# shinshoji01/Style-Restricted_GAN

Hardware: AMD Instinct MI355X
Metric: images/sec G+D+E train step, CelebA 128x128 bs=32/GPU (higher is better)
Workload: dtype f32; 1 GPU; SRGAN-nopretrain (03-train) G+D+E train step, 128x128, bs=32/GPU, k=5, fp32, E trainable (BASELINE configs[1]); global_batch=32, unrolled_k=5, parallelism=dp1, graph_fallback=False, graph_segments=1, ranks_seen=1, execution=hipGraph replay of the captured step

## Files before the change

style-restricted_gan_amd/csrc/conv_igemm.hip:

```cpp
#include <algorithm>
#include <cstdlib>
#include <cstring>
#include <map>
#include <mutex>
#include <string>
#include <vector>
#include "common.h"
#include "pack_device.h"

namespace srgan {

struct ProfSlot { hipEvent_t a, b; int kid; double flops; };
static bool g_prof_on = false;
static std::vector<ProfSlot> g_prof_slots;
static std::vector<std::pair<hipEvent_t, hipEvent_t>> g_prof_pool;
static size_t g_prof_next = 0;
static const char* const kProfNames[] = {
    "igemm_kernel<128,128,2,2,gen>", "igemm_kernel<128,128,2,2,vec>", "igemm_kernel<128,64,2,2,gen>", "igemm_kernel<128,64,2,2,vec>",
    "igemm_kernel<128,32,4,1,gen>",  "igemm_kernel<128,32,4,1,vec>",  "igemm_kernel<64,64,2,2,gen>",  "igemm_kernel<64,64,2,2,vec>",
    "wgrad_kernel<gen>", "wgrad_kernel<vec>", "igemm_kernel<256,128,4,2,gen>", "igemm_kernel<256,128,4,2,vec>",
    "igemm_kernel<256,64,4,2,gen>", "igemm_kernel<256,64,4,2,vec>", "wino_kernel", "wino_wgrad_kernel", "wino_kernel<4x4s2>", "wino_wgrad_kernel<4x4s2>",
    "wino43_kernel", "wino43_input_kernel", "rgbin_conv_kernel", "rgb_wgrad_kernel", "wino43_wgrad_kernel", "wino43_dy_kernel",
    "halo16_kernel", "halo16_wgrad_kernel", "halo16s2_wgrad_kernel", "halo16t_kernel", "rgbout_conv_kernel", "halo16s_kernel",
    "in_stats_partial", "in_apply", "in_bwd_partial", "in_bwd_apply", "in_fwd_slab", "in_bwd_slab", "igemm16_kernel",
// ... 1639 lines not shown
  const long long f = (long long)npad_for(M_f, d->O) * Kf;
  const int s = d->stride;
  const int Ty = (int)ceil_div(d->kh, s), Tx = (int)ceil_div(d->kw, s);
  const long long Kd = round_up((long long)Ty * Tx * d->O, BK);
  const long long g = (long long)s * s * round_up(d->I, 128) * Kd;
  size_t bytes = (size_t)((f > g ? f : g) * sizeof(float));
  if (rowconv_applicable(d)) bytes = std::max(bytes, rowconv_packed_elems(d) * sizeof(float));
  {
    srgan_conv_desc f;
    long long w_off;
    if (narrow_dgrad_desc(d, &f, &w_off) && rowconv_applicable(&f)) bytes = std::max(bytes, rowconv_packed_elems(&f) * sizeof(float));
  }
  if (wino_applicable(d, 0)) bytes = std::max(bytes, wino_packed_bytes(d, 0));
  if (wino_applicable(d, 1)) bytes = std::max(bytes, wino_packed_bytes(d, 1));
  if (d->I == 3 || d->O == 3) bytes = std::max(bytes, (size_t)d->kh * ((d->kw * 3 + 1) & ~1) * std::max(d->I, d->O) * sizeof(float));
  return bytes;
}

}
}

using namespace srgan;

namespace srgan { static size_t conv_splitk_bytes(const srgan_conv_desc* d, int kind); }

extern "C" size_t srgan_conv2d_workspace(const srgan_conv_desc* d) {
  if (validate(d) != 0) return 0;
  size_t bytes = pack_bytes(d);
  if (d->pad_mode == SRGAN_PAD_REFLECT)
    bytes += (size_t)d->N * (d->Hi + 2 * d->pad) * (d->Wi + 2 * d->pad) * d->I * sizeof(float);
  bytes += 256 + std::max(conv_splitk_bytes(d, 0), conv_splitk_bytes(d, 1));
  bytes = std::max(bytes, (size_t)round_up((long long)pack_bytes(d), 256) + std::max(wino_scratch_bytes(d, 0), wino_scratch_bytes(d, 1)));
  WgradPlan w = plan_wgrad(d);
  if (wino_wgrad_applicable(d)) wino_wgrad_slab(d, &w.splits, &w.Cdpad, &w.NNpad);
  if (rgb_wgrad_kind(d) >= 0) rgb_wgrad_slab(d, &w.splits, &w.Cdpad, &w.NNpad);
  size_t wg = (size_t)w.splits * w.Cdpad * w.NNpad * sizeof(float);
  size_t cs = (size_t)1024 * d->O * sizeof(float);
  if (wg + cs > bytes) bytes = wg + cs;
  if (narrow_applicable(d)) bytes = std::max(bytes, narrow_workspace(d) + cs);
  {
    Wino43WgradGeom wg43{};
    if (wino43_wgrad_geometry(d, &wg43)) bytes = std::max(bytes, (size_t)round_up((long long)(wg43.slab_bytes + cs), 256) + wg43.z_bytes);
  }
  return bytes + 4096;
}

namespace srgan {
enum FwdPath { PATH_IGEMM = 0, PATH_NARROW = 1, PATH_WAVE = 2, PATH_DENSE = 3, PATH_WINO = 4, PATH_ROWCONV = 5, PATH_RGBIN = 6 };

static bool rowconv_applicable(const srgan_conv_desc* d) {
  static const bool off = SRGAN_AB_SET("SRGAN_NO_ROWCONV");
  return !off && d->O == 3 && d->kh == 7 && d->kw == 7 && d->stride == 1 && d->pad_mode == SRGAN_PAD_ZERO && (d->I % BK) == 0 &&
         d->Wo >= 64 && d->Ho >= 8 && (long long)d->N * d->Ho * d->Wi * 21 < (1LL << 30);
}
constexpr int RC_N = 21, RC_NPAD = 32;
// ... 322 lines not shown
    long long w_off;
    narrow_dgrad_desc(d, &f, &w_off);
    if (rowconv_applicable(&f)) return rowconv_run(&f, dy, wp, nullptr, dx, st);
    return narrow_fwd_packed(&f, dy, wp, nullptr, dx, st);
  }
  if (g.rgbin) {
    srgan_conv_desc f;
    long long w_off;
    rgbin_dgrad_desc(d, &f, &w_off);
    return rgbin_run(&f, dy, wp, nullptr, dx, SRGAN_ACT_NONE, 0.f, st);
  }
  if (g.narrow_s2) {
    for (int ph = 0; ph < 4; ++ph) {
      srgan_conv_desc f;
      long long w_off;
      int px;
      size_t po;
      if (!narrow_s2_phase(d, ph >> 1, ph & 1, &f, &w_off, &px, &po)) { set_error("narrow stride-2 dgrad: phase geometry"); return -1; }
      if (int e = narrow_fwd_strided(&f, px, dy, wp + po, dx, d->Hi, d->Wi, ph >> 1, ph & 1, st)) return e;
    }
    return 0;
  }
  if (g.wino) {
    if (int e = wino_run(d, 1, dy, wp, nullptr, g.p.dst, SRGAN_ACT_NONE, 0.f, g.reflect ? nullptr : scratch, st,
                         g.reflect ? nullptr : res, res_done, false, (g.reflect || res) ? nullptr : mask, mask_slope, mask_done)) return e;
  } else {
    float* slab = scratch ? (g.reflect ? scratch + round_up((long long)d->N * g.Hd * g.Wd * d->I, 64) : scratch) : nullptr;
    if (int e = run_igemm(g.p, g.phases, st, conv_flops(d), slab)) return e;
  }
  if (g.reflect) {
    long long n = (long long)d->N * d->Hi * d->Wi * d->I;
    hipLaunchKernelGGL(reflect_fold_kernel<false>, dim3((unsigned)std::min<long long>(ceil_div(n, 256), 8192)), dim3(256), 0, st,
                       (const float*)scratch, dx, d->N, d->Hi, d->Wi, d->I, d->pad);
    return check_launch("reflect_fold_kernel");
  }
  return 0;
}
}

extern "C" int srgan_conv2d_fwd(const srgan_conv_desc* d, const float* x, const float* w, const float* bias,
                                float* y, int act, float slope, void* ws, size_t ws_bytes, void* stream) {
  if (int e = validate(d)) return e;
  SRGAN_REQUIRE(x && w && y && ws, "conv2d_fwd: null pointer");
  SRGAN_REQUIRE(ws_bytes >= srgan_conv2d_workspace(d), "conv2d_fwd: workspace too small");
  hipStream_t st = as_stream(stream);
  if (int e = fwd_pack(d, act, w, (float*)ws, st)) return e;
  return fwd_run(d, x, (const float*)ws, bias, y, act, slope, (float*)ws + round_up((long long)(pack_bytes(d) / sizeof(float)), 64), st);
// ... 721 lines not shown
```

style-restricted_gan_amd/csrc/conv_wino.hip:

```cpp
#include <algorithm>
#include <cstdlib>
#include <type_traits>
#include "common.h"
#include "pack_device.h"

#ifndef WINO_EXP
#define WINO_EXP 0
#endif

namespace srgan {

constexpr int WT = 64;
constexpr int WNB = 64;
constexpr int WC = 8;

__device__ __forceinline__ auto uniform_rsrc(const float* base, unsigned bytes) {
  const unsigned long long a = reinterpret_cast<unsigned long long>(base);
  const unsigned lo = __builtin_amdgcn_readfirstlane((unsigned)a), hi = __builtin_amdgcn_readfirstlane((unsigned)(a >> 32));
  float* q = reinterpret_cast<float*>(((unsigned long long)hi << 32) | lo);
  return __builtin_amdgcn_make_buffer_rsrc(q, 0, __builtin_amdgcn_readfirstlane(bytes), 0x00020000);
}



// ... 652 lines not shown
}

static bool wino_disabled() {
  static const bool off = SRGAN_AB_SET("SRGAN_NO_WINOGRAD");
  return off;
}
double wino_threshold_scale() {
  const char* e = std::getenv("SRGAN_WINOGRAD_THRESHOLD_SCALE");
  return e ? std::atof(e) : 1.0;
}
static bool wino43_disabled() {
  static const bool off = SRGAN_AB_SET("SRGAN_NO_WINOGRAD43");
  return off;
}
static bool wino_s2_disabled() {
  static const bool off = SRGAN_AB_SET("SRGAN_NO_WINOGRAD_S2");
  return off;
}
static bool wino42_disabled() {
  static const bool off = SRGAN_AB_SET("SRGAN_NO_WINOGRAD42");
  return off;
}

static int wino_variant(const srgan_conv_desc* d, int kind) {
  if (compute_bf16()) {
    if (halo16_applicable(d, kind)) return 4;
    if (kind == 1 && halo16t_applicable(d)) return 5;
    return kind == 0 && halo16s_applicable(d) ? 6 : 0;
  }
  if (wino_disabled()) return 0;

  const int C = kind == 0 ? d->I : d->O, N = kind == 0 ? d->O : d->I;
  if (C % (2 * WC) != 0 || C < 32 || N < 32 || N % 4 != 0) return 0;
  const long long src_elems = (long long)d->N * (kind == 0 ? (long long)d->Hi * d->Wi * d->I : (long long)d->Ho * d->Wo * d->O);
  if (src_elems >= (1LL << 29)) return 0;
  if (d->kh == 3 && d->kw == 3 && d->stride == 1 && d->pad == 1) {
    if (d->Hi < 3 || d->Wi < 3) return 0;
    const int ho = kind == 0 ? d->Ho : d->Hi, wo = kind == 0 ? d->Wo : d->Wi;
    if (!wino43_disabled() && d->pad_mode == SRGAN_PAD_ZERO && ho % 4 == 0 && wo % 4 == 0 && N % 32 == 0 && C % 32 == 0) {
      const long long b43 = ceil_div((long long)d->N * (ho / 4) * (wo / 4), 64) * (N / 32);
      if (b43 >= 50 * wino_threshold_scale()) return 3;
    }
    const long long blocks = ceil_div((long long)d->N * ceil_div(ho, 2) * ceil_div(wo, 2), WT) * ceil_div(N, WNB);
    return blocks >= 100 * wino_threshold_scale() ? 1 : 0;
  }
  if (d->kh == 4 && d->kw == 4 && d->stride == 2 && d->pad == 1 && d->pad_mode == SRGAN_PAD_ZERO && !wino_s2_disabled()) {
    if ((d->Hi & 1) || (d->Wi & 1)) return 0;
    const long long dst_elems = (long long)d->N * (kind == 0 ? (long long)d->Ho * d->Wo * d->O : (long long)d->Hi * d->Wi * d->I);
    if (!wino42_disabled() && d->Ho % 4 == 0 && d->Wo % 4 == 0 && N % 64 == 0 && C % 16 == 0 && dst_elems < (1LL << 30) &&
        (kind == 1 || C <= 128)) {
      const long long b42 = ceil_div((long long)d->N * (d->Ho / 4) * (d->Wo / 4), 32) * (N / 64) * (kind == 1 ? 4 : 1);
      if (b42 >= 120 * wino_threshold_scale()) return 7;
    }
    const long long th = ceil_div(d->Ho, 3), tw = ceil_div(d->Wo, 3);
    const double eff = (double)d->Ho * d->Wo / (9.0 * th * tw);
    if (eff * 2.25 < 1.5) return 0;
    const long long blocks = ceil_div((long long)d->N * th * tw, WT) * ceil_div(N, WNB) * (kind == 1 ? 4 : 1);
    return blocks >= 120 * wino_threshold_scale() ? 2 : 0;
  }
  return 0;
}

bool wino_applicable(const srgan_conv_desc* d, int kind) { return wino_variant(d, kind) != 0; }

static void wino_dims(const srgan_conv_desc* d, int kind, int* C, int* N, int* n_tiles, int* nchunk, int* phases) {
  const int v = wino_variant(d, kind);
  *C = kind == 0 ? d->I : d->O;
  *N = kind == 0 ? d->O : d->I;
  *n_tiles = v == 7 ? *N / 64 : (v >= 4) ? 1 : v == 3 ? *N / 32 : (int)ceil_div(*N, WNB);
  *nchunk = v == 7 ? (kind == 0 ? 4 : 1) * (*C / 16) : (v >= 4) ? *C / 32 : (v == 2 && kind == 0 ? 4 : 1) * (*C / WC);
  *phases = ((v == 2 || v == 7) && kind == 1) ? 4 : 1;
}

size_t wino_packed_bytes(const srgan_conv_desc* d, int kind) {
  int C, N, n_tiles, nchunk, phases;
  wino_dims(d, kind, &C, &N, &n_tiles, &nchunk, &phases);
  if (wino_variant(d, kind) == 4) return halo16_packed_bytes(d);
  if (wino_variant(d, kind) == 6) return halo16s_packed_bytes(d);
  if (wino_variant(d, kind) == 5) return halo16t_packed_bytes(d);
  if (wino_variant(d, kind) == 3) return (size_t)n_tiles * nchunk * (36 * 256) * sizeof(float);
  if (wino_variant(d, kind) == 7) return (size_t)phases * n_tiles * nchunk * (25 * 1024) * sizeof(float);
  return (size_t)phases * n_tiles * nchunk * 8192 * sizeof(float);
}

size_t wino_scratch_bytes(const srgan_conv_desc* d, int kind) {
  if (wino_variant(d, kind) != 3) return 0;
  const int ho = kind == 0 ? d->Ho : d->Hi, wo = kind == 0 ? d->Wo : d->Wi;
  return wino43_scratch_floats((long long)d->N * (ho / 4) * (wo / 4), kind == 0 ? d->I : d->O) * sizeof(float);
}

bool wino43_wgrad_geometry(const srgan_conv_desc* d, Wino43WgradGeom* g) {
  static const bool off = SRGAN_AB_SET("SRGAN_NO_WINOGRAD43_WGRAD");
  if (off || wino_variant(d, 0) != 3 || d->I % 64 != 0 || d->O % 32 != 0) return false;
  const long long T = (long long)d->N * (d->Ho / 4) * (d->Wo / 4);
  const long long ntc = ceil_div(T, 64) * 8;
  const int tiles = (d->O / 32) * (d->I / 64);
  long long splits = std::max(1, 256 / tiles);
  long long cps = std::max<long long>(2, ceil_div(ntc, splits));
  if (ntc % cps == 1) ++cps;
  splits = ceil_div(ntc, cps);
  if (ntc < 2 || ntc - (splits - 1) * cps < 2) return false;
  g->NB = d->N; g->H = d->Ho; g->W = d->Wo; g->C = d->I; g->O = d->O; g->ntc = (int)ntc;
  g->splits = (int)splits; g->chunks_per_split = (int)cps;
  g->v_bytes = wino_scratch_bytes(d, 0);
  g->z_bytes = (size_t)(d->O / 32) * ntc * 36 * 256 * sizeof(float);
  g->slab_bytes = (size_t)splits * d->O * 9 * d->I * sizeof(float);
  return g->v_bytes < (1ULL << 32) && g->z_bytes < (1ULL << 32);
}

void wino_pack_params(const srgan_conv_desc* d, int kind, const float* w, float* dst, WinoPackParams* out) {
  WinoPackParams q{};
  int C, N;
  wino_dims(d, kind, &C, &N, &q.n_tiles, &q.nchunk, &q.phases);
  q.variant = wino_variant(d, kind);
  q.w = w; q.dst = dst; q.sO = d->sO; q.sI = d->sI; q.sH = d->sH; q.sW = d->sW; q.N = N; q.C = C; q.kind = kind;
  q.no_block = std::getenv("SRGAN_PACK_ITEM_PATH") != nullptr ? 1 : 0;
  *out = q;
}

int wino_pack(const srgan_conv_desc* d, int kind, const float* w, float* dst, hipStream_t st) {
  WinoPackParams q{};
  wino_pack_params(d, kind, w, dst, &q);
  const long long total = wino_pack_total(q);
  hipLaunchKernelGGL(wino_pack_kernel, dim3((unsigned)std::min<long long>(ceil_div(total, 256), 4096)), dim3(256), 0, st, q);
  return check_launch("wino_pack_kernel");
}

bool wino43_fwd_applicable(const srgan_conv_desc* d) { return wino_variant(d, 0) == 3; }
bool wino43_dgrad_applicable(const srgan_conv_desc* d) { return d->pad_mode == SRGAN_PAD_ZERO && wino_variant(d, 1) == 3; }

int wino_run(const srgan_conv_desc* d, int kind, const float* src, const float* packed, const float* bias, float* dst,
             int act, float slope, float* scratch, hipStream_t st, const float* res, bool* res_done, bool v_ready,
             const float* mask, float mask_slope, bool* mask_done) {
  if (res_done) *res_done = false;
  if (mask_done) *mask_done = false;
  WinoParams p{};
  p.act = act; p.slope = slope;
  int C, N, phases;
  wino_dims(d, kind, &C, &N, &p.n_tiles, &p.nchunk, &phases);
  const int variant = wino_variant(d, kind);
  SRGAN_REQUIRE(variant != 0, "winograd: layer not applicable");
  if (variant == 6) {
    SRGAN_REQUIRE(!v_ready && !res && !mask, "halo16s: no prepared image, skip tensor or mask on this path");
    return halo16s_run(d, src, packed, bias, dst, act, slope, conv_flops_of(d), st);
  }
  if (variant == 5) {
    SRGAN_REQUIRE(!v_ready && !bias && act == SRGAN_ACT_NONE, "halo16t: plain transposed product only");
    return halo16t_run(d, src, packed, dst, conv_flops_of(d), st);
  }
  if (variant == 4) {
    SRGAN_REQUIRE(!v_ready, "halo16: no transformed-input image on this path");
    if (res_done) *res_done = res != nullptr;
    return halo16_run(d, kind, src, packed, bias, res, dst, act, slope, conv_flops_of(d), st);
  }
  const bool reflect = d->pad_mode == SRGAN_PAD_REFLECT;
  p.src = src; p.u = packed; p.bias = bias; p.dst = dst;
  p.NB = d->N; p.C = C; p.Cd = N; p.cpp = C / WC;
  int ot = 2;
  if (variant == 1 || variant == 3) {
    if (kind == 0) {
      p.H = d->Hi; p.W = d->Wi; p.Ho = d->Ho; p.Wo = d->Wo; p.pad = d->pad; p.reflect = reflect ? 1 : 0;
    } else {
      p.H = d->Ho; p.W = d->Wo; p.reflect = 0;
      p.pad = reflect ? 2 : 2 - d->pad;
      p.Ho = d->Ho + 2 * p.pad - 2; p.Wo = d->Wo + 2 * p.pad - 2;
    }
    if (variant == 3) { ot = 4; p.TH = p.Ho / 4; p.TW = p.Wo / 4; }
    else { p.TH = (p.Ho + 1) / 2; p.TW = (p.Wo + 1) / 2; }
  } else {
    ot = variant == 7 ? 4 : 3;
    p.pad = d->pad; p.reflect = 0;
    if (kind == 0) { p.H = d->Hi; p.W = d->Wi; p.Ho = d->Ho; p.Wo = d->Wo; }
    else { p.H = d->Ho; p.W = d->Wo; p.Ho = d->Hi; p.Wo = d->Wi; }
    p.TH = (int)ceil_div(d->Ho, ot); p.TW = (int)ceil_div(d->Wo, ot);
    if (variant == 7) p.cpp = C / 16;
  }
  (void)ot;
  const long long T = (long long)p.NB * p.TH * p.TW;
  SRGAN_REQUIRE(T < (1LL << 30), "winograd: too many tiles");
  p.T = (int)T;
  p.m_tiles = (int)ceil_div(T, variant == 7 ? 32 : WT);
  const long long grid = (long long)p.m_tiles * p.n_tiles;
  SRGAN_REQUIRE(grid < (1LL << 31), "winograd: grid too large");
  if (variant == 3) {
    SRGAN_REQUIRE(p.pad == 1 && p.Ho == p.H && p.Wo == p.W && p.nchunk >= 2 && p.Cd % 32 == 0 && p.C % 32 == 0,
                  "winograd F(4,3): geometry");
    SRGAN_REQUIRE(scratch, "winograd F(4,3): no scratch for the transformed input");
    p.res = res;
    if (res_done) *res_done = res != nullptr;
    wino43_launch(p, scratch, grid, conv_flops_of(d), st, v_ready);
    return check_launch("wino43_kernel");
  }
  SRGAN_REQUIRE(!v_ready, "winograd: a prepared V image only serves the F(4x4,3x3) path");
  if (variant == 7) {
    SRGAN_REQUIRE(p.pad == 1 && p.nchunk >= 2 && p.Cd % 64 == 0 && p.C % 16 == 0 && d->Ho % 4 == 0 && d->Wo % 4 == 0, "winograd F(4,2): geometry");
    if (kind == 1 && mask) {
      p.mask = mask; p.mask_slope = mask_slope;
      if (mask_done) *mask_done = true;
    }
    return wino42_launch(p, kind, grid, kind == 1 && mask != nullptr, conv_flops_of(d), st);
  }
  ProfToken tok = prof_begin(variant == 1 ? 14 : 16, conv_flops_of(d), st);
  if (variant == 1) hipLaunchKernelGGL(wino_kernel<0>, dim3((unsigned)grid), dim3(512), 0, st, p);
  else if (kind == 0) hipLaunchKernelGGL(wino_kernel<1>, dim3((unsigned)grid), dim3(512), 0, st, p);
  else if (mask) {
    p.mask = mask; p.mask_slope = mask_slope;
    if (mask_done) *mask_done = true;
    hipLaunchKernelGGL((wino_kernel<2, true>), dim3((unsigned)grid, 4), dim3(512), 0, st, p);
  } else hipLaunchKernelGGL(wino_kernel<2>, dim3((unsigned)grid, 4), dim3(512), 0, st, p);
  prof_end(tok, st);
  return check_launch("wino_kernel");
}
// ... 88 lines not shown
```

style-restricted_gan_amd/csrc/conv_wino43.hip:

```cpp
#include <algorithm>
#include <cstdlib>
#include <type_traits>
#include "common.h"
#include "pack_device.h"

namespace srgan {

__device__ __forceinline__ void bt6(f32x4& x0, f32x4& x1, f32x4& x2, f32x4& x3, f32x4& x4, f32x4& x5) {
  const f32x4 a = x4 - 4.f * x2, b = x3 - 4.f * x1, c = x4 - x2, e = x3 - x1;
  const f32x4 n0 = 4.f * x0 - 5.f * x2 + x4, n5 = 4.f * x1 - 5.f * x3 + x5;
  x0 = n0; x1 = a + b; x2 = a - b; x3 = c + 2.f * e; x4 = c - 2.f * e; x5 = n5;
}

__device__ __forceinline__ void at6(float m0, float m1, float m2, float m3, float m4, float m5, float* y) {
  const float s1 = m1 + m2, d1 = m1 - m2, s2 = m3 + m4, d2 = m3 - m4;
  y[0] = m0 + s1 + s2;
  y[1] = d1 + 2.f * d2;
  y[2] = s1 + 4.f * s2;
  y[3] = d1 + 8.f * d2 + m5;
}

__device__ __forceinline__ auto uniform_rsrc43(const float* base, unsigned bytes) {
  const unsigned long long a = reinterpret_cast<unsigned long long>(base);
  const unsigned lo = __builtin_amdgcn_readfirstlane((unsigned)a), hi = __builtin_amdgcn_readfirstlane((unsigned)(a >> 32));
  float* q = reinterpret_cast<float*>(((unsigned long long)hi << 32) | lo);
  return __builtin_amdgcn_make_buffer_rsrc(q, 0, __builtin_amdgcn_readfirstlane(bytes), 0x00020000);
}

constexpr int W4T = 64;
constexpr int W4N = 32;
constexpr int W4C = 8;
constexpr int W4BLK = 36 * 512;

__global__ __launch_bounds__(512) void wino43_input_kernel(WinoParams p, float* vimg) {
  const int tid = threadIdx.x, lane = tid & 63, wave = tid >> 6;
  const int cgs = p.C / 32;
  int m_tile, cg;
  if ((p.m_tiles & 7) == 0) {
    const int xcd = blockIdx.x & 7, k = blockIdx.x >> 3;
    cg = k % cgs;
    m_tile = (k / cgs) * 8 + xcd;
  } else {
    m_tile = blockIdx.x / cgs;
    cg = blockIdx.x - m_tile * cgs;
  }
  const int quad = lane & 7, tl = wave * 8 + (lane >> 3);
  const int t = m_tile * W4T + tl;
  const bool tv = t < p.T;
  const int tt = tv ? t : 0;
  const int per = p.TH * p.TW;
  const int nb = tt / per;
  const int r0 = tt - nb * per;
  const int ty = r0 / p.TW, tx = r0 - ty * p.TW;
  const int Y = 4 * ty, X = 4 * tx;
  const int RS = p.W * p.C * 4, CS = p.C * 4;
  const auto rs_x = uniform_rsrc43(p.src, (unsigned)((size_t)p.NB * p.H * p.W * p.C * 4));
  constexpr unsigned kOutside = 0x80000000u;
  const unsigned base = (unsigned)(((nb * p.H + Y) * p.W + X) * p.C + cg * 32 + quad * 4) * 4u;
  const bool rok[3] = {Y > 0, true, Y + 4 < p.H};
  const bool cok[3] = {X > 0, true, X + 4 < p.W};
  const int rdl[3] = {-RS, 0, RS}, cdl[3] = {-CS, 0, CS};
  unsigned voff[3][3];
#pragma unroll
  for (int a = 0; a < 3; ++a)
#pragma unroll
    for (int b = 0; b < 3; ++b) voff[a][b] = (tv && rok[a] && cok[b]) ? (unsigned)((int)base + rdl[a] + cdl[b]) : kOutside;
  f32x4 d[6][6];
#pragma unroll
  for (int r = 0; r < 6; ++r)
#pragma unroll
    for (int c = 0; c < 6; ++c) {
      const int rc = r == 0 ? 0 : (r == 5 ? 2 : 1), cc = c == 0 ? 0 : (c == 5 ? 2 : 1);
      const int rs = (r < 1 ? 0 : (r > 4 ? 3 : r - 1)), cs = (c < 1 ? 0 : (c > 4 ? 3 : c - 1));
      d[r][c] = __builtin_bit_cast(f32x4, __builtin_amdgcn_raw_buffer_load_b128(rs_x, voff[rc][cc], rs * RS + cs * CS, 0));
    }
#pragma unroll
  for (int c = 0; c < 6; ++c) bt6(d[0][c], d[1][c], d[2][c], d[3][c], d[4][c], d[5][c]);
  float* out = vimg + ((size_t)m_tile * p.nchunk + cg * 4 + (quad >> 1)) * W4BLK + (quad & 1) * 256 + tl * 4;
#pragma unroll
  for (int r = 0; r < 6; ++r) {
    bt6(d[r][0], d[r][1], d[r][2], d[r][3], d[r][4], d[r][5]);
#pragma unroll
    for (int c = 0; c < 6; ++c) *reinterpret_cast<f32x4*>(out + (r * 6 + c) * 512) = d[r][c];
  }
}

template <int NW>
__device__ __forceinline__ f32x4 slab_sum43_q4(f32x4 v, f32x4 (*sh)[4], int q, int wave) {
#pragma unroll
  for (int o = 4; o < 64; o <<= 1)
#pragma unroll
    for (int e = 0; e < 4; ++e) v[e] += __shfl_xor(v[e], o, 64);
  __syncthreads();
  if ((threadIdx.x & 63) < 4) sh[wave][q] = v;
  __syncthreads();
  f32x4 t = sh[0][q];
#pragma unroll
  for (int w = 1; w < NW; ++w) t += sh[w][q];
// ... 190 lines not shown
      }
    }
    const int ntc = N * 8;
    const int zlane = lh * 32 + (slab & 1) * 16 + o16;
    float* out = zimg + ((size_t)((slab >> 1) * ntc + n * 8 + tc) * 36) * 256 + zlane * 4;
#pragma unroll
    for (int k = 0; k < 36; ++k) {
      const f32x4 v = {z[k][0], z[k][1], z[k][2], z[k][3]};
      *reinterpret_cast<f32x4*>(out + k * 256) = v;
    }
  }
}

int in_bwd_slab_vz_launch(const float* x, const float* gup, const float* scale, const float* shift, const float* mean,
                          const float* rstd, float* dscale, float* dshift, float* vimg, float* zimg, int N, int C, int act,
                          float slope, hipStream_t st) {
  ProfToken tok = prof_begin(39, 6.5 * 4.0 * N * 1024.0 * C, st);
  hipLaunchKernelGGL(in_bwd_slab_vz_kernel, dim3((unsigned)(N * (C / 16))), dim3(256), 0, st, x, gup, scale, shift, mean, rstd, dscale,
                     dshift, vimg, zimg, N, C, act, slope);
  prof_end(tok, st);
  return check_launch("in_bwd_slab_vz_kernel");
}

template <bool RES>
__global__ __launch_bounds__(512) void wino43_kernel(WinoParams p, const float* vimg) {
  constexpr int VH = 64 * 4 + 16, VP = 2 * VH, VSZ = 36 * VP;
  constexpr int XT = 36, XP = 16 * XT;
  static_assert(36 * XP <= 2 * VSZ, "epilogue image must fit the V buffers");
  __shared__ __attribute__((aligned(16))) float lds[2 * VSZ];
  __shared__ int tile_o[W4T];

  const int tid = threadIdx.x, lane = tid & 63, wave = __builtin_amdgcn_readfirstlane(tid >> 6);
  const int lr = lane & 31, lh = lane >> 5;
  int bid = blockIdx.x;
  const int nblk = gridDim.x;
  if ((nblk & 7) == 0) bid = (bid & 7) * (nblk >> 3) + (bid >> 3);
  const int m_tile = bid / p.n_tiles, n_tile = bid - m_tile * p.n_tiles;
  const int nk = p.nchunk;

  const auto rs_v = uniform_rsrc43(vimg + (size_t)m_tile * p.nchunk * W4BLK, (unsigned)p.nchunk * (W4BLK * 4u));
  const auto rs_u = uniform_rsrc43(p.u + (size_t)n_tile * p.nchunk * (36 * 256), (unsigned)p.nchunk * (36u * 1024u));

  if (tid < W4T) {
    const int t = m_tile * W4T + tid;
    int o = -1;
    if (t < p.T) {
      const int per = p.TH * p.TW;
      const int nb = t / per;
      const int r0 = t - nb * per;
      const int ty = r0 / p.TW, tx = r0 - ty * p.TW;
      o = (nb * p.Ho + 4 * ty) * p.Wo + 4 * tx;
    }
    tile_o[tid] = o;
  }
  f32x4 stage[9];
  const int vst = (tid >> 7) * VP + ((tid >> 6) & 1) * VH + (tid & 63) * 4;
  auto load_v1 = [&](int kc, int j) __attribute__((always_inline)) {
    stage[j] = __builtin_bit_cast(f32x4, __builtin_amdgcn_raw_buffer_load_b128(rs_v, tid * 16, kc * (W4BLK * 4) + j * 8192, 0));
  };
  auto store_v1 = [&](int buf, int j) __attribute__((always_inline)) {
    *reinterpret_cast<f32x4*>(lds + buf * VSZ + vst + j * 4 * VP) = stage[j];
  };
  auto load_v = [&](int kc) __attribute__((always_inline)) {
#pragma unroll
    for (int j = 0; j < 9; ++j) load_v1(kc, j);
  };
  auto store_v = [&](int buf) __attribute__((always_inline)) {
#pragma unroll
    for (int j = 0; j < 9; ++j) store_v1(buf, j);
  };

  auto role = [&](auto odd_c) __attribute__((always_inline)) {
    constexpr int ODD = decltype(odd_c)::value;
    const int pbase = (9 * wave) >> 1;
// ... 62 lines not shown
#endif
    }
#ifdef W43_DIAG
    {
      const long long t_loop = __builtin_amdgcn_s_memtime() - t_begin;
      if (blockIdx.x == 17 && lane == 0) {
        float* o = p.dst + wave * 8;
        o[0] = (float)t_loop; o[1] = (float)t_cp; o[2] = (float)t_mm; o[3] = (float)t_bar; o[4] = (float)(nk - 2);
      }
      float keep = 0.f;
#pragma unroll
      for (int i = 0; i < 9; ++i)
#pragma unroll
        for (int e = 0; e < 16; ++e) keep += acc[i][e];
      p.dst[4096 + (size_t)blockIdx.x * 512 + tid] = keep;
      return;
    }
#endif
    mma_chunk(kc, T{}, T{}, F{});
    __syncthreads();
    mma_chunk(kc + 1, F{}, F{}, F{});
    __syncthreads();

    const int ec = lane & 31, et = wave + 8 * (lane >> 5);
    const int n = n_tile * W4N + ec;
    const float bv = p.bias ? p.bias[n] : 0.f;
#pragma unroll
    for (int q = 0; q < 4; ++q) {
      if (q > 0) __syncthreads();
      float rv[16];
      if constexpr (RES) {
        const int eo_r = tile_o[16 * q + et];
        const float* rp = p.res + (size_t)(eo_r >= 0 ? eo_r : 0) * p.Cd + n;
#pragma unroll
        for (int a = 0; a < 4; ++a)
#pragma unroll
          for (int b = 0; b < 4; ++b) rv[a * 4 + b] = eo_r >= 0 ? rp[(size_t)(a * p.Wo + b) * p.Cd] : 0.f;
      }
#pragma unroll
      for (int i = 0; i < 9; ++i) {
        const int g = i + ODD, a = g >> 1, h = g & 1;
        if (h == (q >> 1) && (lr >> 4) == (q & 1)) {
          float* X = lds + (pbase + a) * XP + (lr & 15) * XT + lh * 4;
#pragma unroll
          for (int k = 0; k < 4; ++k) {
            const f32x4 v = {acc[i][4 * k + 0], acc[i][4 * k + 1], acc[i][4 * k + 2], acc[i][4 * k + 3]};
            *reinterpret_cast<f32x4*>(X + 8 * k) = v;
          }
        }
      }
      __syncthreads();
      const float* M = lds + et * XT + ec;
      float hh[4][6];
#pragma unroll
      for (int c = 0; c < 6; ++c) {
        float y[4];
        at6(M[(0 * 6 + c) * XP], M[(1 * 6 + c) * XP], M[(2 * 6 + c) * XP], M[(3 * 6 + c) * XP], M[(4 * 6 + c) * XP],
            M[(5 * 6 + c) * XP], y);
#pragma unroll
        for (int a = 0; a < 4; ++a) hh[a][c] = y[a];
      }
      const int eo = tile_o[16 * q + et];
      if (eo >= 0) {
        float* dp = p.dst + (size_t)eo * p.Cd + n;
        if constexpr (RES) {
#pragma unroll
          for (int a = 0; a < 4; ++a) {
            float y[4];
            at6(hh[a][0], hh[a][1], hh[a][2], hh[a][3], hh[a][4], hh[a][5], y);
#pragma unroll
            for (int b = 0; b < 4; ++b) dp[(size_t)(a * p.Wo + b) * p.Cd] = apply_act(y[b] + bv, p.act, p.slope) + rv[a * 4 + b];
          }
        } else {
#pragma unroll
          for (int a = 0; a < 4; ++a) {
            float y[4];
            at6(hh[a][0], hh[a][1], hh[a][2], hh[a][3], hh[a][4], hh[a][5], y);
#pragma unroll
            for (int b = 0; b < 4; ++b) dp[(size_t)(a * p.Wo + b) * p.Cd] = apply_act(y[b] + bv, p.act, p.slope);
          }
        }
      }
    }
  };

  if (wave & 1) role(std::integral_constant<int, 1>{});
  else role(std::integral_constant<int, 0>{});
}

struct Wino43WgradParams {
  const float* vimg;
  const float* zimg;
  float* slab;
  int C, O, cchunks, ntc, chunks_per_split, splits, c_blocks, o_blocks;
  int split_minor;
};

struct Wino43DyParams {
  const float* dy;
  float* zimg;
  int NB, H, W, O, TH, TW, T, ntc, o_blocks;
};

__global__ __launch_bounds__(512) void wino43_dy_kernel(Wino43DyParams p) {
  const int tid = threadIdx.x, lane = tid & 63, wave = tid >> 6;
  const long long unit = (long long)blockIdx.x * 8 + wave;
  if (unit >= (long long)p.ntc * p.o_blocks) return;
  const int o_blk = (int)(unit % p.o_blocks), tchunk = (int)(unit / p.o_blocks);
  const int o = o_blk * 32 + (lane & 31), lh = lane >> 5;
  const auto rs = uniform_rsrc43(p.dy, (unsigned)((size_t)p.NB * p.H * p.W * p.O * 4));
  float z[36][4];
#pragma unroll
  for (int j = 0; j < 4; ++j) {
    const int t = tchunk * 8 + lh * 4 + j;
    const bool tv = t < p.T;
    const int tt = tv ? t : 0;
    const int per = p.TH * p.TW;
    const int nb = tt / per;
    const int r0 = tt - nb * per;
    const int ty = r0 / p.TW, tx = r0 - ty * p.TW;
    const unsigned base = tv ? (unsigned)(((nb * p.H + 4 * ty) * p.W + 4 * tx) * p.O + o) * 4u : 0x80000000u;
    float e[4][4];
#pragma unroll
    for (int a = 0; a < 4; ++a)
#pragma unroll
      for (int b = 0; b < 4; ++b)
        e[a][b] = __builtin_bit_cast(float, __builtin_amdgcn_raw_buffer_load_b32(rs, base, (a * p.W + b) * p.O * 4, 0));
    float h[6][4];
#pragma unroll
    for (int b = 0; b < 4; ++b) {
      const float v0 = e[0][b], v1 = e[1][b], v2 = e[2][b], v3 = e[3][b];
      const float s02 = v0 + v2, s13 = v1 + v3, q02 = v0 + 4.f * v2, q13 = 2.f * v1 + 8.f * v3;
      h[0][b] = v0; h[1][b] = s02 + s13; h[2][b] = s02 - s13; h[3][b] = q02 + q13; h[4][b] = q02 - q13; h[5][b] = v3;
    }
#pragma unroll
    for (int r = 0; r < 6; ++r) {
      const float v0 = h[r][0], v1 = h[r][1], v2 = h[r][2], v3 = h[r][3];
      const float s02 = v0 + v2, s13 = v1 + v3, q02 = v0 + 4.f * v2, q13 = 2.f * v1 + 8.f * v3;
      z[r * 6 + 0][j] = v0; z[r * 6 + 1][j] = s02 + s13; z[r * 6 + 2][j] = s02 - s13;
      z[r * 6 + 3][j] = q02 + q13; z[r * 6 + 4][j] = q02 - q13; z[r * 6 + 5][j] = v3;
    }
  }
  float* out = p.zimg + ((size_t)(o_blk * p.ntc + tchunk) * 36) * 256 + lane * 4;
#pragma unroll
  for (int k = 0; k < 36; ++k) {
    const f32x4 v = {z[k][0], z[k][1], z[k][2], z[k][3]};
    *reinterpret_cast<f32x4*>(out + k * 256) = v;
  }
}

// ... 109 lines not shown
        const float s12 = m1 + m2, d12 = m2 - m1, s34 = m3 + m4, d34 = m3 - m4;
        t[0][c] = 0.25f * m0 - (1.f / 6.f) * s12 + (1.f / 24.f) * s34;
        t[1][c] = (1.f / 6.f) * d12 + (1.f / 12.f) * d34;
        t[2][c] = -(1.f / 6.f) * s12 + (1.f / 6.f) * s34 + m5;
      }
      float* dst = slab + (size_t)(8 * k + eo) * (9 * p.C);
#pragma unroll
      for (int a = 0; a < 3; ++a) {
        const float s12 = t[a][1] + t[a][2], d12 = t[a][2] - t[a][1], s34 = t[a][3] + t[a][4], d34 = t[a][3] - t[a][4];
        dst[(a * 3 + 0) * p.C] = 0.25f * t[a][0] - (1.f / 6.f) * s12 + (1.f / 24.f) * s34;
        dst[(a * 3 + 1) * p.C] = (1.f / 6.f) * d12 + (1.f / 12.f) * d34;
        dst[(a * 3 + 2) * p.C] = -(1.f / 6.f) * s12 + (1.f / 6.f) * s34 + t[a][5];
      }
    }
  };
  if (wave & 1) role(std::integral_constant<int, 1>{});
  else role(std::integral_constant<int, 0>{});
}

size_t wino43_scratch_floats(long long T, int C) { return (size_t)ceil_div(T, (long long)W4T) * (C / W4C) * W4BLK; }

int wino43_launch(const WinoParams& p, float* vimg, long long grid, double flops, hipStream_t st, bool v_ready) {
  static const int only = SRGAN_AB_INT("SRGAN_W43_ONLY", 0);
  if (only != 2 && !v_ready) {
    ProfToken tok = prof_begin(19, 0.0, st);
    hipLaunchKernelGGL(wino43_input_kernel, dim3((unsigned)(p.m_tiles * (p.C / 32))), dim3(512), 0, st, p, vimg);
    prof_end(tok, st);
  }
  if (only != 1) {
    ProfToken tok = prof_begin(18, flops, st);
    if (p.res) hipLaunchKernelGGL(wino43_kernel<true>, dim3((unsigned)grid), dim3(512), 0, st, p, (const float*)vimg);
    else hipLaunchKernelGGL(wino43_kernel<false>, dim3((unsigned)grid), dim3(512), 0, st, p, (const float*)vimg);
    prof_end(tok, st);
  }
  return 0;
}

int wino43_wgrad_launch(const Wino43WgradGeom& g, const float* vimg, const float* dy, float* zimg, float* slab, double flops,
                        hipStream_t st, bool z_ready) {
  Wino43DyParams q{};
  q.dy = dy; q.zimg = zimg; q.NB = g.NB; q.H = g.H; q.W = g.W; q.O = g.O; q.TH = g.H / 4; q.TW = g.W / 4;
  q.T = g.NB * q.TH * q.TW; q.ntc = g.ntc; q.o_blocks = g.O / 32;
  if (!z_ready) {
    ProfToken tok = prof_begin(23, 0.0, st);
    hipLaunchKernelGGL(wino43_dy_kernel, dim3((unsigned)ceil_div((long long)q.ntc * q.o_blocks, 8)), dim3(512), 0, st, q);
    prof_end(tok, st);
  }
  Wino43WgradParams p{};
  p.vimg = vimg; p.zimg = zimg; p.slab = slab; p.C = g.C; p.O = g.O; p.cchunks = g.C / 8; p.ntc = g.ntc;
  p.chunks_per_split = g.chunks_per_split; p.splits = g.splits; p.c_blocks = g.C / 64; p.o_blocks = g.O / 32;
  p.split_minor = 1;
  ProfToken tok = prof_begin(22, flops, st);
  hipLaunchKernelGGL(wino43_wgrad_kernel, dim3((unsigned)(p.o_blocks * p.c_blocks * p.splits)), dim3(512), 0, st, p);
  prof_end(tok, st);
  return 0;
}

}
```

Measured before the change: 526.6 images/sec.

## Extend Winograd F(4,3) to reflect-padded dgrad and ragged tile shapes

Lets the F(4,3) Winograd path run for reflect-padded convolution data-gradients and for spatial sizes not divisible by 4. It adds a generic input-transform kernel that gathers reflected or zero-padded taps, a ragged epilogue that masks partial output tiles, and a masked dy transform for the weight gradient. Convolutions that used to fall back to F(2,3) or implicit GEMM now take the cheaper-arithmetic path, in exchange for extra workspace and some wasted work on partial tiles. Reflect dgrad writes to a padded scratch that is then folded back.

After: 526.8 images/sec (median of 5 runs). Within noise of the previous version (+0.0%).

```diff
diff --git a/style-restricted_gan_amd/csrc/conv_igemm.hip b/style-restricted_gan_amd/csrc/conv_igemm.hip
--- a/style-restricted_gan_amd/csrc/conv_igemm.hip
+++ b/style-restricted_gan_amd/csrc/conv_igemm.hip
@@ -1685,7 +1685,16 @@
 
 using namespace srgan;
 
-namespace srgan { static size_t conv_splitk_bytes(const srgan_conv_desc* d, int kind); }
+namespace srgan {
+static size_t conv_splitk_bytes(const srgan_conv_desc* d, int kind);
+static long long reflect_wino43_v_offset(const srgan_conv_desc* d) {
+  return round_up((long long)d->N * (d->Hi + 2 * d->pad) * (d->Wi + 2 * d->pad) * d->I, 64);
+}
+static size_t reflect_wino43_scratch_bytes(const srgan_conv_desc* d) {
+  if (d->pad_mode != SRGAN_PAD_REFLECT || !wino43_dgrad_applicable(d)) return 0;
+  return (size_t)reflect_wino43_v_offset(d) * sizeof(float) + wino_scratch_bytes(d, 1);
+}
+}
 
 extern "C" size_t srgan_conv2d_workspace(const srgan_conv_desc* d) {
   if (validate(d) != 0) return 0;
@@ -1694,6 +1703,7 @@
     bytes += (size_t)d->N * (d->Hi + 2 * d->pad) * (d->Wi + 2 * d->pad) * d->I * sizeof(float);
   bytes += 256 + std::max(conv_splitk_bytes(d, 0), conv_splitk_bytes(d, 1));
   bytes = std::max(bytes, (size_t)round_up((long long)pack_bytes(d), 256) + std::max(wino_scratch_bytes(d, 0), wino_scratch_bytes(d, 1)));
+  bytes = std::max(bytes, (size_t)round_up((long long)pack_bytes(d), 256) + reflect_wino43_scratch_bytes(d));
   WgradPlan w = plan_wgrad(d);
   if (wino_wgrad_applicable(d)) wino_wgrad_slab(d, &w.splits, &w.Cdpad, &w.NNpad);
   if (rgb_wgrad_kind(d) >= 0) rgb_wgrad_slab(d, &w.splits, &w.Cdpad, &w.NNpad);
@@ -2062,7 +2072,8 @@
     return 0;
   }
   if (g.wino) {
-    if (int e = wino_run(d, 1, dy, wp, nullptr, g.p.dst, SRGAN_ACT_NONE, 0.f, g.reflect ? nullptr : scratch, st,
+    float* vimg = g.reflect ? (wino43_dgrad_applicable(d) ? scratch + reflect_wino43_v_offset(d) : nullptr) : scratch;
+    if (int e = wino_run(d, 1, dy, wp, nullptr, g.p.dst, SRGAN_ACT_NONE, 0.f, vimg, st,
                          g.reflect ? nullptr : res, res_done, false, (g.reflect || res) ? nullptr : mask, mask_slope, mask_done)) return e;
   } else {
     float* slab = scratch ? (g.reflect ? scratch + round_up((long long)d->N * g.Hd * g.Wd * d->I, 64) : scratch) : nullptr;
diff --git a/style-restricted_gan_amd/csrc/conv_wino.hip b/style-restricted_gan_amd/csrc/conv_wino.hip
--- a/style-restricted_gan_amd/csrc/conv_wino.hip
+++ b/style-restricted_gan_amd/csrc/conv_wino.hip
@@ -698,6 +698,10 @@
   return off;
 }
 
+static int wino43_dst_side(const srgan_conv_desc* d, int kind, int side) {
+  return kind == 1 && d->pad_mode == SRGAN_PAD_REFLECT ? side + 2 * d->pad : side;
+}
+
 static int wino_variant(const srgan_conv_desc* d, int kind) {
   if (compute_bf16()) {
     if (halo16_applicable(d, kind)) return 4;
@@ -713,8 +717,10 @@
   if (d->kh == 3 && d->kw == 3 && d->stride == 1 && d->pad == 1) {
     if (d->Hi < 3 || d->Wi < 3) return 0;
     const int ho = kind == 0 ? d->Ho : d->Hi, wo = kind == 0 ? d->Wo : d->Wi;
-    if (!wino43_disabled() && d->pad_mode == SRGAN_PAD_ZERO && ho % 4 == 0 && wo % 4 == 0 && N % 32 == 0 && C % 32 == 0) {
-      const long long b43 = ceil_div((long long)d->N * (ho / 4) * (wo / 4), 64) * (N / 32);
+    const bool exact = d->pad_mode == SRGAN_PAD_ZERO && ho % 4 == 0 && wo % 4 == 0;
+    if (!wino43_disabled() && (exact || std::min(ho, wo) >= 8) && N % 32 == 0 && C % 32 == 0) {
+      const int th = wino43_dst_side(d, kind, ho), tw = wino43_dst_side(d, kind, wo);
+      const long long b43 = ceil_div((long long)d->N * ceil_div(th, 4) * ceil_div(tw, 4), 64) * (N / 32);
       if (b43 >= 50 * wino_threshold_scale()) return 3;
     }
     const long long blocks = ceil_div((long long)d->N * ceil_div(ho, 2) * ceil_div(wo, 2), WT) * ceil_div(N, WNB);
@@ -761,14 +767,14 @@
 
 size_t wino_scratch_bytes(const srgan_conv_desc* d, int kind) {
   if (wino_variant(d, kind) != 3) return 0;
-  const int ho = kind == 0 ? d->Ho : d->Hi, wo = kind == 0 ? d->Wo : d->Wi;
-  return wino43_scratch_floats((long long)d->N * (ho / 4) * (wo / 4), kind == 0 ? d->I : d->O) * sizeof(float);
+  const int ho = wino43_dst_side(d, kind, kind == 0 ? d->Ho : d->Hi), wo = wino43_dst_side(d, kind, kind == 0 ? d->Wo : d->Wi);
+  return wino43_scratch_floats((long long)d->N * ceil_div(ho, 4) * ceil_div(wo, 4), kind == 0 ? d->I : d->O) * sizeof(float);
 }
 
 bool wino43_wgrad_geometry(const srgan_conv_desc* d, Wino43WgradGeom* g) {
   static const bool off = SRGAN_AB_SET("SRGAN_NO_WINOGRAD43_WGRAD");
   if (off || wino_variant(d, 0) != 3 || d->I % 64 != 0 || d->O % 32 != 0) return false;
-  const long long T = (long long)d->N * (d->Ho / 4) * (d->Wo / 4);
+  const long long T = (long long)d->N * ceil_div(d->Ho, 4) * ceil_div(d->Wo, 4);
   const long long ntc = ceil_div(T, 64) * 8;
   const int tiles = (d->O / 32) * (d->I / 64);
   long long splits = std::max(1, 256 / tiles);
@@ -803,7 +809,7 @@
 }
 
 bool wino43_fwd_applicable(const srgan_conv_desc* d) { return wino_variant(d, 0) == 3; }
-bool wino43_dgrad_applicable(const srgan_conv_desc* d) { return d->pad_mode == SRGAN_PAD_ZERO && wino_variant(d, 1) == 3; }
+bool wino43_dgrad_applicable(const srgan_conv_desc* d) { return wino_variant(d, 1) == 3; }
 
 int wino_run(const srgan_conv_desc* d, int kind, const float* src, const float* packed, const float* bias, float* dst,
              int act, float slope, float* scratch, hipStream_t st, const float* res, bool* res_done, bool v_ready,
@@ -841,7 +847,7 @@
       p.pad = reflect ? 2 : 2 - d->pad;
       p.Ho = d->Ho + 2 * p.pad - 2; p.Wo = d->Wo + 2 * p.pad - 2;
     }
-    if (variant == 3) { ot = 4; p.TH = p.Ho / 4; p.TW = p.Wo / 4; }
+    if (variant == 3) { ot = 4; p.TH = (p.Ho + 3) / 4; p.TW = (p.Wo + 3) / 4; }
     else { p.TH = (p.Ho + 1) / 2; p.TW = (p.Wo + 1) / 2; }
   } else {
     ot = variant == 7 ? 4 : 3;
@@ -859,11 +865,13 @@
   const long long grid = (long long)p.m_tiles * p.n_tiles;
   SRGAN_REQUIRE(grid < (1LL << 31), "winograd: grid too large");
   if (variant == 3) {
-    SRGAN_REQUIRE(p.pad == 1 && p.Ho == p.H && p.Wo == p.W && p.nchunk >= 2 && p.Cd % 32 == 0 && p.C % 32 == 0,
-                  "winograd F(4,3): geometry");
+    SRGAN_REQUIRE(p.Ho == p.H + 2 * p.pad - 2 && p.Wo == p.W + 2 * p.pad - 2 && (p.pad == 1 || (kind == 1 && reflect && p.pad == 2)) &&
+                  p.nchunk >= 2 && p.Cd % 32 == 0 && p.C % 32 == 0, "winograd F(4,3): geometry");
     SRGAN_REQUIRE(scratch, "winograd F(4,3): no scratch for the transformed input");
-    p.res = res;
-    if (res_done) *res_done = res != nullptr;
+    if (p.Ho % 4 == 0 && p.Wo % 4 == 0) {
+      p.res = res;
+      if (res_done) *res_done = res != nullptr;
+    }
     wino43_launch(p, scratch, grid, conv_flops_of(d), st, v_ready);
     return check_launch("wino43_kernel");
   }
diff --git a/style-restricted_gan_amd/csrc/conv_wino43.hip b/style-restricted_gan_amd/csrc/conv_wino43.hip
--- a/style-restricted_gan_amd/csrc/conv_wino43.hip
+++ b/style-restricted_gan_amd/csrc/conv_wino43.hip
@@ -32,6 +32,7 @@
 constexpr int W4C = 8;
 constexpr int W4BLK = 36 * 512;
 
+template <bool GEN>
 __global__ __launch_bounds__(512) void wino43_input_kernel(WinoParams p, float* vimg) {
   const int tid = threadIdx.x, lane = tid & 63, wave = tid >> 6;
   const int cgs = p.C / 32;
@@ -56,24 +57,53 @@
   const int RS = p.W * p.C * 4, CS = p.C * 4;
   const auto rs_x = uniform_rsrc43(p.src, (unsigned)((size_t)p.NB * p.H * p.W * p.C * 4));
   constexpr unsigned kOutside = 0x80000000u;
-  const unsigned base = (unsigned)(((nb * p.H + Y) * p.W + X) * p.C + cg * 32 + quad * 4) * 4u;
-  const bool rok[3] = {Y > 0, true, Y + 4 < p.H};
-  const bool cok[3] = {X > 0, true, X + 4 < p.W};
-  const int rdl[3] = {-RS, 0, RS}, cdl[3] = {-CS, 0, CS};
-  unsigned voff[3][3];
-#pragma unroll
-  for (int a = 0; a < 3; ++a)
-#pragma unroll
-    for (int b = 0; b < 3; ++b) voff[a][b] = (tv && rok[a] && cok[b]) ? (unsigned)((int)base + rdl[a] + cdl[b]) : kOutside;
   f32x4 d[6][6];
-#pragma unroll
-  for (int r = 0; r < 6; ++r)
-#pragma unroll
-    for (int c = 0; c < 6; ++c) {
-      const int rc = r == 0 ? 0 : (r == 5 ? 2 : 1), cc = c == 0 ? 0 : (c == 5 ? 2 : 1);
-      const int rs = (r < 1 ? 0 : (r > 4 ? 3 : r - 1)), cs = (c < 1 ? 0 : (c > 4 ? 3 : c - 1));
-      d[r][c] = __builtin_bit_cast(f32x4, __builtin_amdgcn_raw_buffer_load_b128(rs_x, voff[rc][cc], rs * RS + cs * CS, 0));
-    }
+  if constexpr (!GEN) {
+    const unsigned base = (unsigned)(((nb * p.H + Y) * p.W + X) * p.C + cg * 32 + quad * 4) * 4u;
+    const bool rok[3] = {Y > 0, true, Y + 4 < p.H};
+    const bool cok[3] = {X > 0, true, X + 4 < p.W};
+    const int rdl[3] = {-RS, 0, RS}, cdl[3] = {-CS, 0, CS};
+    unsigned voff[3][3];
+#pragma unroll
+    for (int a = 0; a < 3; ++a)
+#pragma unroll
+      for (int b = 0; b < 3; ++b) voff[a][b] = (tv && rok[a] && cok[b]) ? (unsigned)((int)base + rdl[a] + cdl[b]) : kOutside;
+#pragma unroll
+    for (int r = 0; r < 6; ++r)
+#pragma unroll
+      for (int c = 0; c < 6; ++c) {
+        const int rc = r == 0 ? 0 : (r == 5 ? 2 : 1), cc = c == 0 ? 0 : (c == 5 ? 2 : 1);
+        const int rs = (r < 1 ? 0 : (r > 4 ? 3 : r - 1)), cs = (c < 1 ? 0 : (c > 4 ? 3 : c - 1));
+        d[r][c] = __builtin_bit_cast(f32x4, __builtin_amdgcn_raw_buffer_load_b128(rs_x, voff[rc][cc], rs * RS + cs * CS, 0));
+      }
+  } else {
+    const unsigned base = (unsigned)((nb * p.H * p.W) * p.C + cg * 32 + quad * 4) * 4u;
+    unsigned ro[6], co[6];
+    bool ri[6], ci[6];
+#pragma unroll
+    for (int k = 0; k < 6; ++k) {
+      int yy = Y - p.pad + k, xx = X - p.pad + k;
+      if (p.reflect) {
+        yy = yy < 0 ? -yy : yy;
+        yy = yy >= p.H ? 2 * p.H - 2 - yy : yy;
+        yy = min(max(yy, 0), p.H - 1);
+        xx = xx < 0 ? -xx : xx;
+        xx = xx >= p.W ? 2 * p.W - 2 - xx : xx;
+        xx = min(max(xx, 0), p.W - 1);
+      }
+      ri[k] = (unsigned)yy < (unsigned)p.H;
+      ci[k] = (unsigned)xx < (unsigned)p.W;
+      ro[k] = (unsigned)(yy * RS);
+      co[k] = (unsigned)(xx * CS);
+    }
+#pragma unroll
+    for (int r = 0; r < 6; ++r)
+#pragma unroll
+      for (int c = 0; c < 6; ++c) {
+        const unsigned off = (tv && ri[r] && ci[c]) ? base + ro[r] + co[c] : kOutside;
+        d[r][c] = __builtin_bit_cast(f32x4, __builtin_amdgcn_raw_buffer_load_b128(rs_x, off, 0, 0));
+      }
+  }
 #pragma unroll
   for (int c = 0; c < 6; ++c) bt6(d[0][c], d[1][c], d[2][c], d[3][c], d[4][c], d[5][c]);
   float* out = vimg + ((size_t)m_tile * p.nchunk + cg * 4 + (quad >> 1)) * W4BLK + (quad & 1) * 256 + tl * 4;
@@ -310,8 +340,9 @@
   return check_launch("in_bwd_slab_vz_kernel");
 }
 
-template <bool RES>
+template <bool RES, bool RAG = false>
 __global__ __launch_bounds__(512) void wino43_kernel(WinoParams p, const float* vimg) {
+  static_assert(!(RES && RAG), "the residual add rides on exact tiles only");
   constexpr int VH = 64 * 4 + 16, VP = 2 * VH, VSZ = 36 * VP;
   constexpr int XT = 36, XP = 16 * XT;
   static_assert(36 * XP <= 2 * VSZ, "epilogue image must fit the V buffers");
@@ -338,6 +369,7 @@
       const int r0 = t - nb * per;
       const int ty = r0 / p.TW, tx = r0 - ty * p.TW;
       o = (nb * p.Ho + 4 * ty) * p.Wo + 4 * tx;
+      if constexpr (RAG) o += ((min(4, p.Ho - 4 * ty) - 1) << 26) + ((min(4, p.Wo - 4 * tx) - 1) << 28);
     }
     tile_o[tid] = o;
   }
@@ -446,62 +478,113 @@
     mma_chunk(kc + 1, F{}, F{}, F{});
     __syncthreads();
 
-    const int ec = lane & 31, et = wave + 8 * (lane >> 5);
-    const int n = n_tile * W4N + ec;
-    const float bv = p.bias ? p.bias[n] : 0.f;
-#pragma unroll
-    for (int q = 0; q < 4; ++q) {
-      if (q > 0) __syncthreads();
-      float rv[16];
-      if constexpr (RES) {
-        const int eo_r = tile_o[16 * q + et];
-        const float* rp = p.res + (size_t)(eo_r >= 0 ? eo_r : 0) * p.Cd + n;
-#pragma unroll
-        for (int a = 0; a < 4; ++a)
-#pragma unroll
-          for (int b = 0; b < 4; ++b) rv[a * 4 + b] = eo_r >= 0 ? rp[(size_t)(a * p.Wo + b) * p.Cd] : 0.f;
-      }
-#pragma unroll
-      for (int i = 0; i < 9; ++i) {
-        const int g = i + ODD, a = g >> 1, h = g & 1;
-        if (h == (q >> 1) && (lr >> 4) == (q & 1)) {
-          float* X = lds + (pbase + a) * XP + (lr & 15) * XT + lh * 4;
-#pragma unroll
-          for (int k = 0; k < 4; ++k) {
-            const f32x4 v = {acc[i][4 * k + 0], acc[i][4 * k + 1], acc[i][4 * k + 2], acc[i][4 * k + 3]};
-            *reinterpret_cast<f32x4*>(X + 8 * k) = v;
+    if constexpr (RAG) {
+      int etid = tid;
+      asm volatile("" : "+v"(etid));
+      const int elr = etid & 31, elh = (etid >> 5) & 1;
+      const int ec = elr, et = wave + 8 * elh;
+      const int n = n_tile * W4N + ec;
+      const float bv = p.bias ? p.bias[n] : 0.f;
+#pragma unroll
+      for (int q = 0; q < 4; ++q) {
+        if (q > 0) __syncthreads();
+#pragma unroll
+        for (int i = 0; i < 9; ++i) {
+          const int g = i + ODD, a = g >> 1, h = g & 1;
+          if (h == (q >> 1) && (elr >> 4) == (q & 1)) {
+            float* X = lds + (pbase + a) * XP + (elr & 15) * XT + elh * 4;
+#pragma unroll
+            for (int k = 0; k < 4; ++k) {
+              const f32x4 v = {acc[i][4 * k + 0], acc[i][4 * k + 1], acc[i][4 * k + 2], acc[i][4 * k + 3]};
+              *reinterpret_cast<f32x4*>(X + 8 * k) = v;
+            }
           }
         }
-      }
-      __syncthreads();
-      const float* M = lds + et * XT + ec;
-      float hh[4][6];
-#pragma unroll
-      for (int c = 0; c < 6; ++c) {
-        float y[4];
-        at6(M[(0 * 6 + c) * XP], M[(1 * 6 + c) * XP], M[(2 * 6 + c) * XP], M[(3 * 6 + c) * XP], M[(4 * 6 + c) * XP],
-            M[(5 * 6 + c) * XP], y);
-#pragma unroll
-        for (int a = 0; a < 4; ++a) hh[a][c] = y[a];
-      }
-      const int eo = tile_o[16 * q + et];
-      if (eo >= 0) {
-        float* dp = p.dst + (size_t)eo * p.Cd + n;
+        __syncthreads();
+        const float* M = lds + et * XT + ec;
+        float hh[4][6];
+#pragma unroll
+        for (int c = 0; c < 6; ++c) {
+          float y[4];
+          at6(M[(0 * 6 + c) * XP], M[(1 * 6 + c) * XP], M[(2 * 6 + c) * XP], M[(3 * 6 + c) * XP], M[(4 * 6 + c) * XP],
+              M[(5 * 6 + c) * XP], y);
+#pragma unroll
+          for (int a = 0; a < 4; ++a) hh[a][c] = y[a];
+        }
+        const int eo_m = tile_o[16 * q + et];
+        if (eo_m >= 0) {
+          float* dp = p.dst + (size_t)(eo_m & ((1 << 26) - 1)) * p.Cd + n;
+          const int vr = ((eo_m >> 26) & 3) + 1, vc = (eo_m >> 28) + 1;
+#pragma unroll
+          for (int a = 0; a < 4; ++a) {
+            if (a < vr) {
+              float y[4];
+              at6(hh[a][0], hh[a][1], hh[a][2], hh[a][3], hh[a][4], hh[a][5], y);
+#pragma unroll
+              for (int b = 0; b < 4; ++b)
+                if (b < vc) dp[(size_t)(a * p.Wo + b) * p.Cd] = apply_act(y[b] + bv, p.act, p.slope);
+            }
+          }
+        }
+      }
+    } else {
+      const int ec = lane & 31, et = wave + 8 * (lane >> 5);
+      const int n = n_tile * W4N + ec;
+      const float bv = p.bias ? p.bias[n] : 0.f;
+#pragma unroll
+      for (int q = 0; q < 4; ++q) {
+        if (q > 0) __syncthreads();
+        float rv[16];
         if constexpr (RES) {
-#pragma unroll
-          for (int a = 0; a < 4; ++a) {
-            float y[4];
-            at6(hh[a][0], hh[a][1], hh[a][2], hh[a][3], hh[a][4], hh[a][5], y);
-#pragma unroll
-            for (int b = 0; b < 4; ++b) dp[(size_t)(a * p.Wo + b) * p.Cd] = apply_act(y[b] + bv, p.act, p.slope) + rv[a * 4 + b];
+          const int eo_r = tile_o[16 * q + et];
+          const float* rp = p.res + (size_t)(eo_r >= 0 ? eo_r : 0) * p.Cd + n;
+#pragma unroll
+          for (int a = 0; a < 4; ++a)
+#pragma unroll
+            for (int b = 0; b < 4; ++b) rv[a * 4 + b] = eo_r >= 0 ? rp[(size_t)(a * p.Wo + b) * p.Cd] : 0.f;
+        }
+#pragma unroll
+        for (int i = 0; i < 9; ++i) {
+          const int g = i + ODD, a = g >> 1, h = g & 1;
+          if (h == (q >> 1) && (lr >> 4) == (q & 1)) {
+            float* X = lds + (pbase + a) * XP + (lr & 15) * XT + lh * 4;
+#pragma unroll
+            for (int k = 0; k < 4; ++k) {
+              const f32x4 v = {acc[i][4 * k + 0], acc[i][4 * k + 1], acc[i][4 * k + 2], acc[i][4 * k + 3]};
+              *reinterpret_cast<f32x4*>(X + 8 * k) = v;
+            }
           }
-        } else {
-#pragma unroll
-          for (int a = 0; a < 4; ++a) {
-            float y[4];
-            at6(hh[a][0], hh[a][1], hh[a][2], hh[a][3], hh[a][4], hh[a][5], y);
-#pragma unroll
-            for (int b = 0; b < 4; ++b) dp[(size_t)(a * p.Wo + b) * p.Cd] = apply_act(y[b] + bv, p.act, p.slope);
+        }
+        __syncthreads();
+        const float* M = lds + et * XT + ec;
+        float hh[4][6];
+#pragma unroll
+        for (int c = 0; c < 6; ++c) {
+          float y[4];
+          at6(M[(0 * 6 + c) * XP], M[(1 * 6 + c) * XP], M[(2 * 6 + c) * XP], M[(3 * 6 + c) * XP], M[(4 * 6 + c) * XP],
+              M[(5 * 6 + c) * XP], y);
+#pragma unroll
+          for (int a = 0; a < 4; ++a) hh[a][c] = y[a];
+        }
+        const int eo = tile_o[16 * q + et];
+        if (eo >= 0) {
+          float* dp = p.dst + (size_t)eo * p.Cd + n;
+          if constexpr (RES) {
+#pragma unroll
+            for (int a = 0; a < 4; ++a) {
+              float y[4];
+              at6(hh[a][0], hh[a][1], hh[a][2], hh[a][3], hh[a][4], hh[a][5], y);
+#pragma unroll
+              for (int b = 0; b < 4; ++b) dp[(size_t)(a * p.Wo + b) * p.Cd] = apply_act(y[b] + bv, p.act, p.slope) + rv[a * 4 + b];
+            }
+          } else {
+#pragma unroll
+            for (int a = 0; a < 4; ++a) {
+              float y[4];
+              at6(hh[a][0], hh[a][1], hh[a][2], hh[a][3], hh[a][4], hh[a][5], y);
+#pragma unroll
+              for (int b = 0; b < 4; ++b) dp[(size_t)(a * p.Wo + b) * p.Cd] = apply_act(y[b] + bv, p.act, p.slope);
+            }
           }
         }
       }
@@ -526,6 +609,7 @@
   int NB, H, W, O, TH, TW, T, ntc, o_blocks;
 };
 
+template <bool RAG>
 __global__ __launch_bounds__(512) void wino43_dy_kernel(Wino43DyParams p) {
   const int tid = threadIdx.x, lane = tid & 63, wave = tid >> 6;
   const long long unit = (long long)blockIdx.x * 8 + wave;
@@ -548,8 +632,10 @@
 #pragma unroll
     for (int a = 0; a < 4; ++a)
 #pragma unroll
-      for (int b = 0; b < 4; ++b)
-        e[a][b] = __builtin_bit_cast(float, __builtin_amdgcn_raw_buffer_load_b32(rs, base, (a * p.W + b) * p.O * 4, 0));
+      for (int b = 0; b < 4; ++b) {
+        const unsigned off = (!RAG || (4 * ty + a < p.H && 4 * tx + b < p.W)) ? base : 0x80000000u;
+        e[a][b] = __builtin_bit_cast(float, __builtin_amdgcn_raw_buffer_load_b32(rs, off, (a * p.W + b) * p.O * 4, 0));
+      }
     float h[6][4];
 #pragma unroll
     for (int b = 0; b < 4; ++b) {
@@ -705,14 +791,19 @@
 
 int wino43_launch(const WinoParams& p, float* vimg, long long grid, double flops, hipStream_t st, bool v_ready) {
   static const int only = SRGAN_AB_INT("SRGAN_W43_ONLY", 0);
+  const bool exact = p.pad == 1 && !p.reflect && p.Ho == p.H && p.Wo == p.W && p.H % 4 == 0 && p.W % 4 == 0;
+  const bool ragged = p.Ho % 4 != 0 || p.Wo % 4 != 0;
   if (only != 2 && !v_ready) {
     ProfToken tok = prof_begin(19, 0.0, st);
-    hipLaunchKernelGGL(wino43_input_kernel, dim3((unsigned)(p.m_tiles * (p.C / 32))), dim3(512), 0, st, p, vimg);
+    const dim3 grid_in((unsigned)(p.m_tiles * (p.C / 32)));
+    if (exact) hipLaunchKernelGGL(wino43_input_kernel<false>, grid_in, dim3(512), 0, st, p, vimg);
+    else hipLaunchKernelGGL(wino43_input_kernel<true>, grid_in, dim3(512), 0, st, p, vimg);
     prof_end(tok, st);
   }
   if (only != 1) {
     ProfToken tok = prof_begin(18, flops, st);
     if (p.res) hipLaunchKernelGGL(wino43_kernel<true>, dim3((unsigned)grid), dim3(512), 0, st, p, (const float*)vimg);
+    else if (ragged) hipLaunchKernelGGL((wino43_kernel<false, true>), dim3((unsigned)grid), dim3(512), 0, st, p, (const float*)vimg);
     else hipLaunchKernelGGL(wino43_kernel<false>, dim3((unsigned)grid), dim3(512), 0, st, p, (const float*)vimg);
     prof_end(tok, st);
   }
@@ -722,11 +813,13 @@
 int wino43_wgrad_launch(const Wino43WgradGeom& g, const float* vimg, const float* dy, float* zimg, float* slab, double flops,
                         hipStream_t st, bool z_ready) {
   Wino43DyParams q{};
-  q.dy = dy; q.zimg = zimg; q.NB = g.NB; q.H = g.H; q.W = g.W; q.O = g.O; q.TH = g.H / 4; q.TW = g.W / 4;
+  q.dy = dy; q.zimg = zimg; q.NB = g.NB; q.H = g.H; q.W = g.W; q.O = g.O; q.TH = (g.H + 3) / 4; q.TW = (g.W + 3) / 4;
   q.T = g.NB * q.TH * q.TW; q.ntc = g.ntc; q.o_blocks = g.O / 32;
   if (!z_ready) {
     ProfToken tok = prof_begin(23, 0.0, st);
-    hipLaunchKernelGGL(wino43_dy_kernel, dim3((unsigned)ceil_div((long long)q.ntc * q.o_blocks, 8)), dim3(512), 0, st, q);
+    const dim3 grid_dy((unsigned)ceil_div((long long)q.ntc * q.o_blocks, 8));
+    if (g.H % 4 == 0 && g.W % 4 == 0) hipLaunchKernelGGL(wino43_dy_kernel<false>, grid_dy, dim3(512), 0, st, q);
+    else hipLaunchKernelGGL(wino43_dy_kernel<true>, grid_dy, dim3(512), 0, st, q);
     prof_end(tok, st);
   }
   Wino43WgradParams p{};
```
